# ylongqi/openrec

Hardware: NVIDIA H100
Metric: bpr_triplets_per_sec (higher is better)
Workload: dtype f32

## Files before the change

### include/orx.h

```cpp
#ifndef ORX_H_
#define ORX_H_

#include <stdint.h>

#ifdef __cplusplus
extern "C" {
#endif

#define ORX_ABI_VERSION 1
#define ORX_API __attribute__((visibility("default")))

typedef struct orx_ctx* orx_handle_t;
typedef void* orx_stream_t;

enum orx_status {
  ORX_OK = 0,
  ORX_ERR_INVALID = -1,
  ORX_ERR_CUDA = -2,
  ORX_ERR_UNSUPPORTED = -3,
  ORX_ERR_NOMEM = -4
};

enum orx_pair_kind { ORX_PAIR_BPR = 0, ORX_PAIR_UCML = 1 };
enum orx_point_kind { ORX_POINT_GMF = 0, ORX_POINT_WRMF = 1 };
// ... 26 lines not shown
  ORX_OP_GEMM = 0,
  ORX_OP_INTERACT_FWD = 1,
  ORX_OP_INTERACT_BWD = 2,
  ORX_OP_PAIRWISE_STEP = 3,
  ORX_OP_POINTWISE_STEP = 4,
  ORX_OP_SCORE_RANK = 5,
  ORX_OP_SCORE_TOPK = 6,
  ORX_OP_SCORE_RANK_SHARD = 7
};
enum orx_dispatch_variant {
  ORX_VARIANT_GEMM_TMA = 0,
  ORX_VARIANT_GEMM_SIMT = 1,
  ORX_VARIANT_INTERACT_WARP = 2,
  ORX_VARIANT_INTERACT = 3,
  ORX_VARIANT_STEP = 4,
  ORX_VARIANT_STEP_PIPE = 5,
  ORX_VARIANT_STEP_GENERIC = 6,
  ORX_VARIANT_RANK_SMEM = 7,
  ORX_VARIANT_RANK_GLOBAL = 8,
  ORX_VARIANT_TOPK = 9
};
#define ORX_DISPATCH_LOG_CAP 64
ORX_API int orx_debug_dispatch_log(orx_handle_t h, int32_t* rec_host, int32_t cap, int32_t* n_host);

ORX_API int orx_profile_enable(orx_handle_t h, int32_t on);
ORX_API int orx_profile_read(orx_handle_t h, float* ms_host, int32_t n_phases, int32_t* n_steps_host);

ORX_API int orx_fill_uniform(orx_handle_t h, float* dst, int64_t n, float lo, float hi, uint64_t seed, orx_stream_t s);
ORX_API int orx_gather(orx_handle_t h, const float* tab, int64_t rows, int32_t dim, const void* ids, int32_t id_is_i64,
               int64_t n, float* out, int32_t* n_bad, orx_stream_t s);
ORX_API int orx_censor(orx_handle_t h, float* tab, int64_t rows, int32_t dim, const int32_t* ids, int32_t n,
               float min_norm, orx_stream_t s);

ORX_API int orx_pairwise_step(orx_handle_t h, int32_t kind, const orx_table_t* user, const orx_table_t* item,
                      const orx_table_t* item_bias, const int32_t* uid, const int32_t* pid, const int32_t* nid,
                      int32_t B, float margin, float c_loss, float c_l2, const orx_opt_t* opt_host,
                      float* out4, orx_stream_t s);
ORX_API int orx_pairwise_step_host(orx_handle_t h, int32_t kind, const orx_table_t* user, const orx_table_t* item,
                           const orx_table_t* item_bias, const int32_t* uid_host, const int32_t* pid_host,
                           const int32_t* nid_host, int32_t B, float margin, float c_loss, float c_l2,
                           const orx_opt_t* opt_host, float* out4_host, orx_stream_t s);
ORX_API int orx_pairwise_prefetch(orx_handle_t h, const orx_table_t* user, const orx_table_t* item, const int32_t* uid,
                                  const int32_t* pid, const int32_t* nid, int32_t B, int32_t opt_kind, int32_t ids_ready,
                                  orx_stream_t ids_stream);
ORX_API int orx_pairwise_fwd(orx_handle_t h, int32_t kind, const orx_table_t* user, const orx_table_t* item,
                     const orx_table_t* item_bias, const int32_t* uid, const int32_t* pid, const int32_t* nid,
// ... 124 lines not shown
```

### openrec_b200/_lib.py

```python
from __future__ import annotations

import ctypes as C
import os

HERE = os.path.dirname(os.path.abspath(__file__))
LIB_PATH = os.path.join(HERE, "csrc", "liborx.so")

ORX_PAIR_BPR, ORX_PAIR_UCML = 0, 1
ORX_POINT_GMF, ORX_POINT_WRMF = 0, 1
ORX_SCORE_DOT, ORX_SCORE_NEG_SQDIST = 0, 1
ORX_OPT_SGD, ORX_OPT_ADAGRAD, ORX_OPT_ADAM_LAZY, ORX_OPT_ADAM_DENSE = 0, 1, 2, 3
ORX_OP_GEMM, ORX_OP_INTERACT_FWD, ORX_OP_INTERACT_BWD, ORX_OP_PAIRWISE_STEP, ORX_OP_POINTWISE_STEP = 0, 1, 2, 3, 4
ORX_OP_SCORE_RANK, ORX_OP_SCORE_TOPK, ORX_OP_SCORE_RANK_SHARD = 5, 6, 7
ORX_VARIANT_GEMM_TMA, ORX_VARIANT_GEMM_SIMT, ORX_VARIANT_INTERACT_WARP, ORX_VARIANT_INTERACT = 0, 1, 2, 3
ORX_VARIANT_STEP, ORX_VARIANT_STEP_PIPE, ORX_VARIANT_STEP_GENERIC = 4, 5, 6
ORX_VARIANT_RANK_SMEM, ORX_VARIANT_RANK_GLOBAL, ORX_VARIANT_TOPK = 7, 8, 9
ORX_MAX_AT = 8
ORX_MAX_TOPK = 1024
ORX_DISPATCH_LOG_CAP = 64


class OrxOpt(C.Structure):
    _fields_ = [("kind", C.c_int32), ("lr", C.c_float), ("eps", C.c_float), ("beta1", C.c_float),
                ("beta2", C.c_float), ("step", C.c_int64)]
# ... 16 lines not shown
                ("local_users", C.c_int64), ("local_items", C.c_int64)]


class OrxSampler(C.Structure):
    _fields_ = [("rec_user", C.c_void_p), ("rec_item", C.c_void_p), ("perm_cur", C.c_void_p), ("perm_next", C.c_void_p),
                ("cursor", C.c_int64), ("n_records", C.c_int64), ("csr_off", C.c_void_p), ("csr_items", C.c_void_p),
                ("total_users", C.c_int32), ("total_items", C.c_int32)]


_vp, _i32, _i64, _f, _u64 = C.c_void_p, C.c_int32, C.c_int64, C.c_float, C.c_uint64
_T = C.POINTER(OrxTable)
_O = C.POINTER(OrxOpt)
_S = C.POINTER(OrxShard)

SIGNATURES = {
    "orx_abi_version": [],
    "orx_last_error_string": [],
    "orx_create": [C.c_int, C.POINTER(_vp)],
    "orx_destroy": [_vp],
    "orx_device_count": [C.POINTER(C.c_int)],
    "orx_stream_synchronize": [_vp, _vp],
    "orx_debug_set_epoch": [_vp, C.c_uint32],
    "orx_debug_dispatch_log": [_vp, C.POINTER(_i32), _i32, C.POINTER(_i32)],
    "orx_profile_enable": [_vp, _i32],
    "orx_profile_read": [_vp, C.POINTER(C.c_float), _i32, C.POINTER(_i32)],
    "orx_fill_uniform": [_vp, _vp, _i64, _f, _f, _u64, _vp],
    "orx_gather": [_vp, _vp, _i64, _i32, _vp, _i32, _i64, _vp, _vp, _vp],
    "orx_censor": [_vp, _vp, _i64, _i32, _vp, _i32, _f, _vp],
    "orx_pairwise_step": [_vp, _i32, _T, _T, _T, _vp, _vp, _vp, _i32, _f, _f, _f, _O, _vp, _vp],
    "orx_pairwise_step_host": [_vp, _i32, _T, _T, _T, _vp, _vp, _vp, _i32, _f, _f, _f, _O, _vp, _vp],
    "orx_pairwise_prefetch": [_vp, _T, _T, _vp, _vp, _vp, _i32, _i32, _i32, _vp],
    "orx_pairwise_fwd": [_vp, _i32, _T, _T, _T, _vp, _vp, _vp, _i32, _f, _vp, _vp],
    "orx_pairwise_grad": [_vp, _i32, _T, _T, _T, _vp, _vp, _vp, _i32, _f, _f, _f, _vp, _vp, _vp, _vp, _vp, _vp, _vp],
    "orx_sparse_apply": [_vp, _T, _vp, _vp, _i32, _O, _vp],
    "orx_sparse_apply_strided": [_vp, _T, _vp, _i64, _vp, _i64, _i32, _O, _vp],
    "orx_gather_strided": [_vp, _vp, _i64, _i32, _vp, _i64, _i64, _vp, _i64, _vp, _vp],
    "orx_mlp_layer_fwd": [_vp, _vp, _i64, _i32, _i32, _vp, _vp, _i32, _i32, _vp, _i64, _vp],
    "orx_mlp_layer_bwd": [_vp, _vp, _i64, _vp, _i64, _vp, _i32, _i32, _i32, _i32, _vp, _i64, _vp, _i64, _vp, _vp, _vp],
    "orx_interact_fwd": [_vp, _vp, _i64, _vp, _i64, _i32, _i32, _i32, _i32, _i32, _vp, _i64, _vp],
    "orx_interact_bwd": [_vp, _vp, _i64, _vp, _i64, _vp, _i64, _i32, _i32, _i32, _i32, _i32, _vp, _i64, _vp, _i64,
                         _vp],
    "orx_pred_loss": [_vp, _vp, _vp, _i32, _i32, _f, _vp, _vp, _vp, _vp],
    "orx_peer_alloc": [_vp, _i64, C.POINTER(_vp), C.c_char_p],
    "orx_peer_open": [_vp, C.c_char_p, C.POINTER(_vp)],
    "orx_peer_close": [_vp, _vp],
    "orx_peer_free": [_vp, _vp],
# ... 51 lines not shown
```

### openrec_b200/csrc/orx_common.cuh

```cuda
#pragma once
#include <cuda_runtime.h>
#include <stdint.h>
#include <stdio.h>

#include <functional>
#include <initializer_list>
#include <type_traits>

#include "../../include/orx.h"

void orx_set_error(const char* fmt, ...);

#define ORX_CUDA(call)                                                                         \
  do {                                                                                         \
    cudaError_t e__ = (call);                                                                  \
    if (e__ != cudaSuccess) {                                                                  \
      orx_set_error("%s:%d %s -> %s", __FILE__, __LINE__, #call, cudaGetErrorString(e__));     \
      return ORX_ERR_CUDA;                                                                     \
    }                                                                                          \
  } while (0)

#define ORX_REQUIRE(cond, msg)                                  \
  do {                                                          \
    if (!(cond)) {                                              \
// ... 21 lines not shown
  OrxHash hu, hi;
  OrxHash pf_u[2], pf_i[2];
  int32_t* counters;
  float *gu, *gi, *gb, *gw;
  int64_t g_rows_u, g_rows_i;
  int32_t g_dim;
  float* partials;
  size_t partials_cap;
  int32_t* ids_stage[2];
  size_t stage_cap[2];
  float* out_stage[2];
  uint32_t stage_flip;
  int prof_on, prof_n, prof_cap;
  int prof_step;
  cudaEvent_t* prof_ev;
  int32_t* bucket_cursor;
  cudaStream_t side_stream;
  cudaEvent_t side_ev;
  cudaEvent_t pf_done[2], pf_free[2], stage_free[2];
  int pf_free_valid[2], stage_free_valid[2];
  int pf_valid, pf_set, pf_next, pf_B, pf_mode;
  const int32_t *pf_uid, *pf_pid, *pf_nid;
  int64_t pf_rows_u, pf_rows_i;
  uint32_t epoch;
  void* shard_ws;
  void* shard_scratch;
  size_t shard_cap;
  int32_t dispatch[ORX_DISPATCH_LOG_CAP][8];
  int64_t dispatch_n;
  void* eval_ws;
  size_t eval_cap;
  float* splitk;
  size_t splitk_cap;
};

int orx_grow(void** buf, size_t* cap, size_t need);

static inline void orx_log_dispatch(orx_ctx* c, int op, int variant, int TA, int TB, int M, int N, int K, int S) {
  int32_t* r = c->dispatch[c->dispatch_n++ % ORX_DISPATCH_LOG_CAP];
  r[0] = op; r[1] = variant; r[2] = TA; r[3] = TB; r[4] = M; r[5] = N; r[6] = K; r[7] = S;
}

int orx_next_epoch(orx_ctx* c, cudaStream_t st);
void orx_shard_ws_release(orx_ctx* c);
bool orx_shard_holds_index(const orx_ctx* c);

// ... 370 lines not shown
        if (!ZERO_ONLY) orx_update1<OPT>(W + e, P0 + e, P1 + e, W[e], G[e], a.opt);
        G[e] = 0.f;
      }
    }
    if (on && !is_u && sl == 0) {
      if (!ZERO_ONLY) orx_update1<OPT>(a.Bv + id, a.Bs0 + id, a.Bs1 + id, a.Bv[id], a.gb[d], a.opt);
      a.gb[d] = 0.f;
    }
  }
}
#endif

OrxOptDev orx_opt_to_dev(const orx_opt_t* o);
int orx_launch_index_build_strided(orx_ctx* c, const int32_t* a, int64_t stride, int64_t rows, int32_t n,
                                   bool stage_all, cudaStream_t st);
SparseArgs orx_sparse_args(const orx_ctx* c, const orx_table_t* user, const orx_table_t* item, const orx_table_t* bias,
                           const OrxHash& hu, const OrxHash& hi, const OrxOptDev& o);
int orx_check_step_tables(const orx_table_t* user, const orx_table_t* item, const orx_table_t* bias,
                          const orx_table_t* w, int opt_kind);
static inline int orx_step_blocks(int B) { return ((B + 7) / 8 + 7) / 8; }
struct OrxStepLaunch {
  int n_partials, variant, minb;
};
typedef std::function<int(const SparseArgs& s, float* partials, OrxStepLaunch* out)> OrxStepKernel;
int orx_sparse_step(orx_ctx* c, int op, int kind, const orx_table_t* user, const orx_table_t* item,
                    const orx_table_t* bias, const orx_table_t* w, const int32_t* uid, const int32_t* iid,
                    const int32_t* nid, int B, const orx_opt_t* opt, float loss_scale, float c_l2, float* out4,
                    const OrxStepKernel& kernel, cudaStream_t st);
int orx_sparse_unfused(orx_ctx* c, int B, float loss_scale, float* out4,
                       const std::function<void(float* partials, int blocks)>& launch, cudaStream_t st);
int orx_launch_adam_sweeps(orx_ctx* c, const orx_table_t* user, const orx_table_t* item, const orx_table_t* bias,
                           const OrxHash& hu, const OrxHash& hi, const OrxOptDev& o, cudaStream_t st);
int orx_launch_tail(orx_ctx* c, const TailArgs& ta, int opt_kind, cudaStream_t st);
int orx_launch_reduce_partials(const float* partials, int n, float loss_scale, float* out4, cudaStream_t st);
int orx_launch_index_build(orx_ctx* c, const int32_t* a, int64_t rows_a, const int32_t* b0, const int32_t* b1,
                           int64_t rows_b, int32_t n, int mode , cudaStream_t st);
```

### openrec_b200/csrc/orx_ctx.cu

```cuda
#include <stdarg.h>
#include <stdlib.h>
#include <string.h>

#include "orx_common.cuh"

static thread_local char g_err[512] = "";

void orx_set_error(const char* fmt, ...) {
  va_list ap;
  va_start(ap, fmt);
  vsnprintf(g_err, sizeof(g_err), fmt, ap);
  va_end(ap);
}

extern "C" const char* orx_last_error_string(void) { return g_err; }

bool orx_pdl_enabled() {
  static int v = -1;
  if (v < 0) {
    const char* e = getenv("ORX_PDL");
    v = (e && atoi(e) == 0) ? 0 : 1;
  }
  return v != 0;
}
// ... 51 lines not shown
  return ORX_OK;
}

int orx_ensure_workspace(orx_ctx* c, int64_t B, int32_t dim) {
  if (B <= c->cap_B && dim <= c->g_dim) return ORX_OK;
  if (orx_shard_holds_index(c)) {
    orx_set_error("workspace growth to %lld lookups / dim %d refused: a sharded step's announced batch holds this "
                  "handle's index sets until its orx_shard_step call", (long long)B, dim);
    return ORX_ERR_INVALID;
  }
  int64_t nb = B > c->cap_B ? B : c->cap_B;
  int32_t nd = dim > c->g_dim ? dim : c->g_dim;
  ORX_CUDA(cudaDeviceSynchronize());
  free_workspace(c);
  int rc;
  if ((rc = alloc_hash(c->hu, nb, c->counters + 0)) != ORX_OK) return rc;
  if ((rc = alloc_hash(c->hi, 2 * nb, c->counters + 1)) != ORX_OK) return rc;
  for (int k = 0; k < 2; ++k) {
    if ((rc = alloc_hash(c->pf_u[k], nb, c->counters + 4 * (1 + k))) != ORX_OK) return rc;
    if ((rc = alloc_hash(c->pf_i[k], 2 * nb, c->counters + 4 * (1 + k) + 1)) != ORX_OK) return rc;
  }
  c->pf_valid = 0;
  c->pf_free_valid[0] = c->pf_free_valid[1] = 0;
  c->g_rows_u = nb;
  c->g_rows_i = 2 * nb;
  size_t bu = sizeof(float) * (size_t)c->g_rows_u * nd, bi = sizeof(float) * (size_t)c->g_rows_i * nd;
  ORX_CUDA(cudaMalloc(&c->gu, bu));
  ORX_CUDA(cudaMalloc(&c->gi, bi));
  ORX_CUDA(cudaMalloc(&c->gb, sizeof(float) * (size_t)c->g_rows_i));
  ORX_CUDA(cudaMalloc(&c->gw, sizeof(float) * (size_t)nd));
  ORX_CUDA(cudaMemset(c->gu, 0, bu));
  ORX_CUDA(cudaMemset(c->gi, 0, bi));
  ORX_CUDA(cudaMemset(c->gb, 0, sizeof(float) * (size_t)c->g_rows_i));
  ORX_CUDA(cudaMemset(c->gw, 0, sizeof(float) * (size_t)nd));
  ORX_CUDA(cudaMemset(c->counters, 0, sizeof(int32_t) * 16));
  ORX_CUDA(cudaDeviceSynchronize());
  c->cap_B = nb;
  c->g_dim = nd;
  c->epoch = 0;
  return ORX_OK;
}

static int zero_hash(OrxHash& t) {
  if (!t.slots) return ORX_OK;
  ORX_CUDA(cudaMemset(t.slots, 0, sizeof(unsigned long long) * ((size_t)t.mask + 1)));
  return ORX_OK;
// ... 52 lines not shown
  *cap = need;
  return ORX_OK;
}

extern "C" int orx_create(int device, orx_handle_t* out) {
  ORX_REQUIRE(out != nullptr, "null output handle");
  *out = nullptr;
  int n = 0;
  ORX_CUDA(cudaGetDeviceCount(&n));
  ORX_REQUIRE(device >= 0 && device < n, "device ordinal out of range");
  ORX_CUDA(cudaSetDevice(device));
  cudaDeviceProp prop;
  ORX_CUDA(cudaGetDeviceProperties(&prop, device));
  if (prop.major != 9 || prop.minor != 0) {
    orx_set_error("orx_create: liborx is built for sm_90a only; device %d is sm_%d%d", device, prop.major,
                  prop.minor);
    return ORX_ERR_UNSUPPORTED;
  }
  orx_ctx* c = new orx_ctx();
  memset(c, 0, sizeof(*c));
  c->device = device;
  c->num_sms = prop.multiProcessorCount;
  c->partials_cap = sizeof(float) * 2 * (size_t)c->num_sms * 64;
  if (cudaMalloc(&c->counters, sizeof(int32_t) * 16) != cudaSuccess ||
      cudaMalloc(&c->bucket_cursor, sizeof(int32_t) * 1024) != cudaSuccess ||
      cudaMalloc(&c->partials, c->partials_cap) != cudaSuccess ||
      cudaMalloc(&c->out_stage[0], sizeof(float) * 8) != cudaSuccess ||
      cudaMalloc(&c->out_stage[1], sizeof(float) * 8) != cudaSuccess) {
    orx_set_error("orx_create: workspace allocation failed: %s", cudaGetErrorString(cudaGetLastError()));
    orx_destroy(c);
    return ORX_ERR_NOMEM;
  }
  cudaMemset(c->counters, 0, sizeof(int32_t) * 16);
  *out = c;
  return ORX_OK;
}

extern "C" int orx_destroy(orx_handle_t h) {
  if (!h) return ORX_OK;
  cudaSetDevice(h->device);
  cudaDeviceSynchronize();
  free_workspace(h);
  for (int i = 0; i < 2; ++i) {
    cudaFree(h->ids_stage[i]);
    cudaFree(h->out_stage[i]);
  }
  cudaFree(h->counters);
  cudaFree(h->partials);
  cudaFree(h->bucket_cursor);
  cudaFree(h->eval_ws);
  cudaFree(h->splitk);
  cudaFree(h->shard_scratch);
  orx_shard_ws_release(h);
  if (h->side_stream) {
    cudaStreamDestroy(h->side_stream);
    cudaEventDestroy(h->side_ev);
    for (int i = 0; i < 2; ++i) {
      cudaEventDestroy(h->pf_done[i]);
      cudaEventDestroy(h->pf_free[i]);
      cudaEventDestroy(h->stage_free[i]);
    }
  }
  if (h->prof_ev) {
    for (int i = 0; i < h->prof_cap * ORX_PROF_EV; ++i) cudaEventDestroy(h->prof_ev[i]);
    delete[] h->prof_ev;
  }
  delete h;
  return ORX_OK;
// ... 60 lines not shown
```

### openrec_b200/csrc/orx_pair.cuh

```cuda
#pragma once
#include "orx_common.cuh"

struct PairArgs : SparseArgs {
  int64_t rowsU, rowsI;
  const int32_t *uid, *pid, *nid;
  int B;
  float margin, c_loss, c_l2, inv_B;
  float* partials;
  float *d_user, *d_pos, *d_neg, *d_bp, *d_bn, *g_out;
  int64_t ld;
};

__device__ __forceinline__ float dot4(float4 a, float4 b) { return a.x * b.x + a.y * b.y + a.z * b.z + a.w * b.w; }
__device__ __forceinline__ float sqd4(float4 a, float4 b) {
  float x = a.x - b.x, y = a.y - b.y, z = a.z - b.z, w = a.w - b.w;
  return x * x + y * y + z * z + w * w;
}
__device__ __forceinline__ float4 axmb_pcd(float s, float4 a, float4 b, float c, float4 d) {
  return make_float4(s * (a.x - b.x) + c * d.x, s * (a.y - b.y) + c * d.y, s * (a.z - b.z) + c * d.z,
                     s * (a.w - b.w) + c * d.w);
}
__device__ __forceinline__ float4 sa_pcd(float s, float4 a, float c, float4 d) {
  return make_float4(s * a.x + c * d.x, s * a.y + c * d.y, s * a.z + c * d.z, s * a.w + c * d.w);
}

template <int KIND>
__device__ __forceinline__ void pair_score(float s1, float s2, float bp, float bn, float margin, float c_loss,
                                           float inv_B, float* loss_term, float* g) {
  if (KIND == ORX_PAIR_BPR) {
    const float x = (s1 + bp) - (s2 + bn);
    const float y = fmaxf(x, -30.f);
// ... 42 lines not shown
```

### openrec_b200/csrc/orx_pairwise.cu

```cuda
#include "orx_common.cuh"
#include "orx_pair.cuh"

__global__ void k_index_build(OrxHash hu, OrxHash hi, const int32_t* __restrict__ a, int64_t rows_a,
                              const int32_t* __restrict__ b0, const int32_t* __restrict__ b1, int64_t rows_b, int n,
                              int stage_all, int32_t* bad) {
  const int i = blockIdx.x * blockDim.x + threadIdx.x;
  if (i >= (b1 ? 3 : 2) * n) return;
  const int t = i < n ? i : (i < 2 * n ? i - n : i - 2 * n);
  const int32_t ia = a[t], ib0 = b0[t], ib1 = b1 ? b1[t] : 0;
  const bool ga = ia >= 0 && (int64_t)ia < rows_a, gb0 = ib0 >= 0 && (int64_t)ib0 < rows_b,
             gb1 = ib1 >= 0 && (int64_t)ib1 < rows_b;
  const bool all = ga && gb0 && gb1;
  if (i < n) {
    if (!ga) atomicAdd(bad, 1);
    else if (all) orx_hash_insert(hu, ia, stage_all);
  } else {
    const bool g = i < 2 * n ? gb0 : gb1;
    if (!g) atomicAdd(bad, 1);
    else if (all) orx_hash_insert(hi, i < 2 * n ? ib0 : ib1, stage_all);
  }
}

__global__ void k_index_build_strided(OrxHash hu, const int32_t* __restrict__ a, int64_t stride, int64_t rows, int n,
                                       int stage_all, int32_t* bad) {
  for (int i = blockIdx.x * blockDim.x + threadIdx.x; i < n; i += gridDim.x * blockDim.x) {
    const int32_t id = a[(int64_t)i * stride];
    if (id >= 0 && (int64_t)id < rows) orx_hash_insert(hu, id, stage_all);
    else atomicAdd(bad, 1);
  }
}

int orx_launch_index_build_strided(orx_ctx* c, const int32_t* a, int64_t stride, int64_t rows, int32_t n,
                                   bool stage_all, cudaStream_t st) {
  if (n <= 0) return ORX_OK;
  int rc = orx_next_epoch(c, st);
  if (rc) return rc;
  k_index_build_strided<<<(n + 255) / 256, 256, 0, st>>>(c->hu, a, stride, rows, n, stage_all ? 1 : 0, c->counters + 3);
  ORX_LAUNCH_CHECK();
  return ORX_OK;
}

int orx_launch_index_build(orx_ctx* c, const int32_t* a, int64_t rows_a, const int32_t* b0, const int32_t* b1,
                           int64_t rows_b, int32_t n, int mode, cudaStream_t st) {
  const int total = (b1 ? 3 : 2) * n;
  if (total <= 0) return ORX_OK;
  int rc = orx_next_epoch(c, st);
  if (rc) return rc;
  k_index_build<<<(total + 255) / 256, 256, 0, st>>>(c->hu, c->hi, a, rows_a, b0, b1, rows_b, n, mode, c->counters + 3);
  ORX_LAUNCH_CHECK();
  return ORX_OK;
}

template <int K, bool S0, bool S1>
struct TripRegs {
  float4 u[K], p[K], n[K];
  float4 us0[K], ps0[K], ns0[K];
  float4 us1[K], ps1[K], ns1[K];
  int fl, uu, pp, nn, du, dp, dn;
  float bp, bn;
};

template <int KIND, int OPT, int D, int CH, int MINB, bool PIPE>
__global__ void __launch_bounds__(256, MINB) k_pair_step(const PairArgs a) {
  constexpr int G = (D / 4 < 32) ? D / 4 : 32;
  constexpr int K = D / (4 * G);
  constexpr int TPW = 32 / G;
  typedef OrxOptSlots<OPT> SL;
  static_assert(CH % TPW == 0, "chunk must be a multiple of the triplets per warp");
  typedef TripRegs<K, SL::S0, SL::S1> Regs;

  const int lane = threadIdx.x & 31;
  const int warp = (blockIdx.x * blockDim.x + threadIdx.x) >> 5;
  const int grp = lane / G, gl = lane % G;
  const int t = warp * CH + lane;
  const float4 z4 = make_float4(0.f, 0.f, 0.f, 0.f);
  orx_pdl_wait();

  int u_id = 0, p_id = 0, n_id = 0, du = -1, dp = -1, dn = -1, flags = 0;
  if (lane < CH && t < a.B) {
    u_id = a.uid[t];
    p_id = a.pid[t];
    n_id = a.nid[t];
    flags = (u_id >= 0 && u_id < a.rowsU && p_id >= 0 && p_id < a.rowsI && n_id >= 0 && n_id < a.rowsI) ? 1 : 0;
  }

  auto load_var = [&](int j, Regs& r) {
    const int src = j + grp;
    r.fl = __shfl_sync(ORX_FULL, flags, src) & 1;
    r.uu = __shfl_sync(ORX_FULL, u_id, src);
    r.pp = __shfl_sync(ORX_FULL, p_id, src);
    r.nn = __shfl_sync(ORX_FULL, n_id, src);
#pragma unroll
    for (int k = 0; k < K; ++k) {
      const int off = (k * G + gl) * 4;
      r.u[k] = r.fl ? orx_ld4_stream(a.U + (int64_t)r.uu * D + off) : z4;
      r.p[k] = r.fl ? orx_ld4_stream(a.I + (int64_t)r.pp * D + off) : z4;
      r.n[k] = r.fl ? orx_ld4_stream(a.I + (int64_t)r.nn * D + off) : z4;
    }
  };
  Regs ra, rb;
  load_var(0, ra);
  if (PIPE && TPW < CH) load_var(TPW, rb);

  float bp = 0.f, bn = 0.f, bps0 = 0.f, bps1 = 0.f, bns0 = 0.f, bns1 = 0.f;
  if (flags & 1) {
    const uint32_t cu = orx_hash_find<!SL::STAGE_ONLY, true>(a.hu, u_id, &du);
    const uint32_t cp = orx_hash_find<!SL::STAGE_ONLY, true>(a.hi, p_id, &dp);
    const uint32_t cn = orx_hash_find<!SL::STAGE_ONLY, true>(a.hi, n_id, &dn);
    bp = orx_ld_keep(a.Bv + p_id);
    bn = orx_ld_keep(a.Bv + n_id);
    if (!SL::STAGE_ONLY) {
      flags |= (cu == 1u ? 2 : 0) | (cp == 1u ? 4 : 0) | (cn == 1u ? 8 : 0);
      if (SL::S0) {
        if (flags & 4) bps0 = orx_ld_keep(a.Bs0 + p_id);
        if (flags & 8) bns0 = orx_ld_keep(a.Bs0 + n_id);
      }
      if (SL::S1) {
        if (flags & 4) bps1 = orx_ld_keep(a.Bs1 + p_id);
        if (flags & 8) bns1 = orx_ld_keep(a.Bs1 + n_id);
      }
    }
  }

  auto load_slots = [&](int j, Regs& r) {
    const int src = j + grp;
    r.fl = __shfl_sync(ORX_FULL, flags, src);
    r.du = __shfl_sync(ORX_FULL, du, src);
    r.dp = __shfl_sync(ORX_FULL, dp, src);
    r.dn = __shfl_sync(ORX_FULL, dn, src);
    r.bp = __shfl_sync(ORX_FULL, bp, src);
    r.bn = __shfl_sync(ORX_FULL, bn, src);
#pragma unroll
    for (int k = 0; k < K; ++k) {
      const int off = (k * G + gl) * 4;
      if (SL::S0) {
        r.us0[k] = (r.fl & 2) ? orx_ld4_stream(a.Us0 + (int64_t)r.uu * D + off) : z4;
        r.ps0[k] = (r.fl & 4) ? orx_ld4_stream(a.Is0 + (int64_t)r.pp * D + off) : z4;
        r.ns0[k] = (r.fl & 8) ? orx_ld4_stream(a.Is0 + (int64_t)r.nn * D + off) : z4;
      }
      if (SL::S1) {
        r.us1[k] = (r.fl & 2) ? orx_ld4_stream(a.Us1 + (int64_t)r.uu * D + off) : z4;
        r.ps1[k] = (r.fl & 4) ? orx_ld4_stream(a.Is1 + (int64_t)r.pp * D + off) : z4;
        r.ns1[k] = (r.fl & 8) ? orx_ld4_stream(a.Is1 + (int64_t)r.nn * D + off) : z4;
      }
    }
  };
  load_slots(0, ra);
  if (PIPE && TPW < CH) load_slots(TPW, rb);

  float loss_acc = 0.f, l2_acc = 0.f, g_own = 0.f;

  auto process = [&](int j, Regs& r) {
    float s1 = 0.f, s2 = 0.f, sq = 0.f;
#pragma unroll
    for (int k = 0; k < K; ++k) {
      if (KIND == ORX_PAIR_BPR) {
        s1 += dot4(r.u[k], r.p[k]);
        s2 += dot4(r.u[k], r.n[k]);
      } else {
        s1 += sqd4(r.u[k], r.p[k]);
        s2 += sqd4(r.u[k], r.n[k]);
      }
      sq += dot4(r.u[k], r.u[k]) + dot4(r.p[k], r.p[k]) + dot4(r.n[k], r.n[k]);
    }
    l2_acc += sq;
    s1 = orx_group_sum<G>(s1);
    s2 = orx_group_sum<G>(s2);
    float lt, g;
    pair_score<KIND>(s1, s2, r.bp, r.bn, a.margin, a.c_loss, a.inv_B, &lt, &g);
    const bool v = r.fl & 1;
    if (!v) { lt = 0.f; g = 0.f; }
    if (gl == 0) loss_acc += lt;
    const float gbias = (KIND == ORX_PAIR_BPR) ? g : -g;
#pragma unroll
    for (int q = 0; q < TPW; ++q) {
      const float val = __shfl_sync(ORX_FULL, gbias, q * G);
      if (lane == j + q) g_own = val;
    }
    if (v) {
#pragma unroll
      for (int k = 0; k < K; ++k) {
        const int off = (k * G + gl) * 4;
        float4 gu, gp, gn;
        pair_row_grads<KIND>(g, a.c_l2, r.u[k], r.p[k], r.n[k], &gu, &gp, &gn);
        orx_own_or_stage4<OPT, true>(r.fl & 2, a.U, a.Us0, a.Us1, r.uu, a.gu, r.du, D, off, r.u[k], gu, r.us0[k],
                                     r.us1[k], a.opt);
        orx_own_or_stage4<OPT, true>(r.fl & 4, a.I, a.Is0, a.Is1, r.pp, a.gi, r.dp, D, off, r.p[k], gp, r.ps0[k],
                                     r.ps1[k], a.opt);
        orx_own_or_stage4<OPT, true>(r.fl & 8, a.I, a.Is0, a.Is1, r.nn, a.gi, r.dn, D, off, r.n[k], gn, r.ns0[k],
                                     r.ns1[k], a.opt);
      }
    }
// ... 290 lines not shown
static int prefetch_drop(orx_ctx* c, cudaStream_t st) {
  if (!c->pf_valid) return ORX_OK;
  const int k = c->pf_set;
  ORX_CUDA(cudaStreamWaitEvent(st, c->pf_done[k], 0));
  ORX_CUDA(cudaMemsetAsync(c->counters + 4 * (1 + k), 0, sizeof(int32_t) * 4, st));
  ORX_CUDA(cudaEventRecord(c->pf_free[k], st));
  c->pf_free_valid[k] = 1;
  c->pf_valid = 0;
  return ORX_OK;
}

static int prefetch_issue(orx_ctx* c, const int32_t* uid, const int32_t* pid, const int32_t* nid, int B, int64_t rows_u,
                          int64_t rows_i, int mode) {
  const int k = c->pf_next;
  c->pf_next ^= 1;
  cudaStream_t ss = c->side_stream;
  if (c->pf_free_valid[k]) ORX_CUDA(cudaStreamWaitEvent(ss, c->pf_free[k], 0));
  int rc = orx_next_epoch(c, ss);
  if (rc) return rc;
  c->pf_u[k].epoch = c->pf_i[k].epoch = c->epoch;
  k_index_build<<<(3 * B + 255) / 256, 256, 0, ss>>>(c->pf_u[k], c->pf_i[k], uid, rows_u, pid, nid, rows_i, B, mode,
                                                     c->counters + 4 * (1 + k) + 3);
  ORX_LAUNCH_CHECK();
  ORX_CUDA(cudaEventRecord(c->pf_done[k], ss));
  c->pf_valid = 1; c->pf_set = k; c->pf_uid = uid; c->pf_pid = pid; c->pf_nid = nid; c->pf_B = B;
  c->pf_rows_u = rows_u; c->pf_rows_i = rows_i; c->pf_mode = mode;
  return ORX_OK;
}

extern "C" int orx_pairwise_prefetch(orx_handle_t h, const orx_table_t* user, const orx_table_t* item, const int32_t* uid,
                                     const int32_t* pid, const int32_t* nid, int32_t B, int32_t opt_kind, int32_t ids_ready,
                                     orx_stream_t ids_stream) {
  ORX_REQUIRE(h != nullptr && user && item && uid && pid && nid && B > 0, "bad arguments");
  ORX_REQUIRE(orx_opt_kind_ok(opt_kind), "unknown optimizer kind");
  ORX_REQUIRE(!orx_shard_holds_index(h), "a sharded step's announced batch holds this handle's index sets (a prefetch "
                                         "would overwrite one) until its orx_shard_step call");
  ORX_CUDA(cudaSetDevice(h->device));
  cudaStream_t is = (cudaStream_t)ids_stream;
  int rc = orx_ensure_workspace(h, B, user->dim);
  if (rc) return rc;
  if ((rc = side_stream_ensure(h))) return rc;
  if ((rc = prefetch_drop(h, is))) return rc;
  if (!ids_ready) {
    ORX_CUDA(cudaEventRecord(h->side_ev, is));
    ORX_CUDA(cudaStreamWaitEvent(h->side_stream, h->side_ev, 0));
  }
  return prefetch_issue(h, uid, pid, nid, B, user->rows, item->rows, opt_kind == ORX_OPT_ADAM_DENSE ? 1 : 0);
}

int orx_sparse_step(orx_ctx* c, int op, int kind, const orx_table_t* user, const orx_table_t* item,
                    const orx_table_t* bias, const orx_table_t* w, const int32_t* uid, const int32_t* iid,
                    const int32_t* nid, int B, const orx_opt_t* opt, float loss_scale, float c_l2, float* out4,
                    const OrxStepKernel& kernel, cudaStream_t st) {
  ORX_REQUIRE(opt != nullptr && out4 != nullptr, "null opt/out");
  ORX_REQUIRE(orx_opt_kind_ok(opt->kind), "unknown optimizer kind");
  ORX_REQUIRE(B > 0 && uid && iid, "empty batch or null ids");
  int rc = orx_check_step_tables(user, item, bias, w, opt->kind);
  if (rc) return rc;
  const int D = user->dim;
  if ((rc = orx_ensure_workspace(c, B, D))) return rc;
  const bool dense = opt->kind == ORX_OPT_ADAM_DENSE;
  if ((rc = orx_grow((void**)&c->partials, &c->partials_cap, sizeof(float) * 2 * 8 * (size_t)orx_step_blocks(B))))
    return rc;
  orx_prof_mark(c, 0, st);
  int set = 0;
  if (nid && c->pf_valid && c->pf_uid == uid && c->pf_pid == iid && c->pf_nid == nid && c->pf_B == B &&
      c->pf_rows_u == user->rows && c->pf_rows_i == item->rows && c->pf_mode == (dense ? 1 : 0)) {
    set = 1 + c->pf_set;
    ORX_CUDA(cudaStreamWaitEvent(st, c->pf_done[c->pf_set], 0));
    c->pf_valid = 0;
  } else {
    if (nid && (rc = prefetch_drop(c, st))) return rc;
    if ((rc = orx_launch_index_build(c, uid, user->rows, iid, nid, item->rows, B, dense ? 1 : 0, st))) return rc;
  }
  const OrxHash& HU = set ? c->pf_u[set - 1] : c->hu;
  const OrxHash& HI = set ? c->pf_i[set - 1] : c->hi;
  orx_prof_mark(c, 1, st);
  const SparseArgs s = orx_sparse_args(c, user, item, bias, HU, HI, orx_opt_to_dev(opt));
  OrxStepLaunch L = {};
  if ((rc = kernel(s, c->partials, &L))) return rc;
  orx_log_dispatch(c, op, L.variant, kind, opt->kind, B, D, L.minb, set);
  orx_prof_mark(c, 2, st);
  if (dense && (rc = orx_launch_adam_sweeps(c, user, item, bias, HU, HI, s.opt, st))) return rc;
  TailArgs ta = {s};
  ta.partials = c->partials; ta.n_partials = L.n_partials; ta.loss_scale = loss_scale;
  ta.counters = c->counters + 4 * set; ta.out4 = out4;
  if (w) {
    ta.W = w->var; ta.Ws0 = w->s0; ta.Ws1 = w->s1; ta.gw = c->gw; ta.c_l2 = c_l2;
  }
  rc = orx_launch_tail(c, ta, opt->kind, st);
  if (set) {
    ORX_CUDA(cudaEventRecord(c->pf_free[set - 1], st));
    c->pf_free_valid[set - 1] = 1;
  }
  orx_prof_mark(c, 3, st);
  orx_prof_next(c);
  return rc;
}

static PairArgs pair_args(const SparseArgs& s, int64_t rows_u, int64_t rows_i, const int32_t* uid, const int32_t* pid,
                          const int32_t* nid, int B, float margin, float c_loss, float c_l2, float inv_B) {
  PairArgs pa = {s};
  pa.rowsU = rows_u; pa.rowsI = rows_i;
  pa.uid = uid; pa.pid = pid; pa.nid = nid; pa.B = B;
  pa.margin = margin; pa.c_loss = c_loss; pa.c_l2 = c_l2; pa.inv_B = inv_B;
  return pa;
}

static int pairwise_step_impl(orx_ctx* c, int kind, const orx_table_t* user, const orx_table_t* item,
                              const orx_table_t* bias, const int32_t* uid, const int32_t* pid, const int32_t* nid,
                              int B, float margin, float c_loss, float c_l2, const orx_opt_t* opt, float* out4,
                              cudaStream_t st) {
  ORX_REQUIRE(kind == ORX_PAIR_BPR || kind == ORX_PAIR_UCML, "unknown pairwise kind");
  ORX_REQUIRE(nid != nullptr, "empty batch or null ids");
  const float inv_B = 1.0f / (float)B;
  const auto kernel = [&](const SparseArgs& s, float* partials, OrxStepLaunch* out) {
    PairArgs pa = pair_args(s, user->rows, item->rows, uid, pid, nid, B, margin, c_loss, c_l2, inv_B);
    pa.partials = partials;
    return orx_dispatch<ORX_PAIR_BPR, ORX_PAIR_UCML>(kind, [&](auto K) {
      return orx_dispatch_opt(opt->kind, [&](auto O) {
        return launch_pair_step_kind_opt<decltype(K)::value, decltype(O)::value>(pa, st, out);
      });
    });
  };
  return orx_sparse_step(c, ORX_OP_PAIRWISE_STEP, kind, user, item, bias, nullptr, uid, pid, nid, B, opt,
                         kind == ORX_PAIR_BPR ? inv_B : 1.0f, c_l2, out4, kernel, st);
}

extern "C" int orx_pairwise_step(orx_handle_t h, int32_t kind, const orx_table_t* user, const orx_table_t* item,
                                 const orx_table_t* item_bias, const int32_t* uid, const int32_t* pid,
                                 const int32_t* nid, int32_t B, float margin, float c_loss, float c_l2,
                                 const orx_opt_t* opt, float* out4, orx_stream_t s) {
  ORX_REQUIRE(h != nullptr, "null handle");
  ORX_CUDA(cudaSetDevice(h->device));
  return pairwise_step_impl(h, kind, user, item, item_bias, uid, pid, nid, B, margin, c_loss, c_l2, opt, out4,
                            (cudaStream_t)s);
}

extern "C" int orx_pairwise_step_host(orx_handle_t h, int32_t kind, const orx_table_t* user, const orx_table_t* item,
                                      const orx_table_t* item_bias, const int32_t* uid_host, const int32_t* pid_host,
                                      const int32_t* nid_host, int32_t B, float margin, float c_loss, float c_l2,
// ... 120 lines not shown
```

### openrec_b200/csrc/orx_pointwise.cu

```cuda
#include "orx_common.cuh"

struct PointArgs : SparseArgs {
  const float* W;
  float* gw;
  int64_t rowsU, rowsI;
  const int32_t *uid, *iid;
  const float* label;
  int B;
  float wa, wb, c_loss, c_l2, inv_B;
  int use_sigmoid;
  float* partials;
  float *d_user, *d_item, *d_bias, *g_out;
};

template <int KIND>
__device__ __forceinline__ void point_score(float s, float bias, float label, const PointArgs& a, float* lt,
                                            float* g) {
  if (KIND == ORX_POINT_GMF) {
    const float z = s + bias;
    *lt = fmaxf(z, 0.f) - z * label + log1pf(expf(-fabsf(z)));
    *g = a.c_loss * (orx_sigmoid(z) - label) * a.inv_B;
  } else {
    float pred = s + bias;
    if (a.use_sigmoid) pred = orx_sigmoid(pred);
// ... 246 lines not shown
                            const orx_table_t* item, const int32_t* uid, const int32_t* iid, const float* label, int B,
                            float a, float b, int use_sigmoid, float c_loss, float c_l2) {
  PointArgs pa = {s};
  pa.W = dense_w ? dense_w->var : nullptr;
  pa.rowsU = user->rows; pa.rowsI = item->rows;
  pa.uid = uid; pa.iid = iid; pa.label = label; pa.B = B;
  pa.wa = a; pa.wb = b; pa.c_loss = c_loss; pa.c_l2 = c_l2; pa.inv_B = 1.0f / (float)B;
  pa.use_sigmoid = use_sigmoid;
  return pa;
}

extern "C" int orx_pointwise_step(orx_handle_t h, int32_t kind, const orx_table_t* user, const orx_table_t* item,
                                  const orx_table_t* item_bias, const orx_table_t* w, const int32_t* uid,
                                  const int32_t* iid, const float* label, int32_t B, float a, float b,
                                  int32_t use_sigmoid, float c_loss, float c_l2, const orx_opt_t* opt, float* out4,
                                  orx_stream_t s) {
  ORX_REQUIRE(h != nullptr, "null handle");
  ORX_REQUIRE(label != nullptr, "empty batch or null inputs");
  ORX_REQUIRE(kind == ORX_POINT_GMF || kind == ORX_POINT_WRMF, "unknown pointwise kind");
  ORX_REQUIRE(kind == ORX_POINT_WRMF || w, "GMF needs w with dim == D");
  const orx_table_t* dense_w = (kind == ORX_POINT_GMF) ? w : nullptr;
  ORX_CUDA(cudaSetDevice(h->device));
  cudaStream_t st = (cudaStream_t)s;
  const auto kernel = [&](const SparseArgs& sa, float* partials, OrxStepLaunch* out) {
    PointArgs pa = point_args(sa, dense_w, user, item, uid, iid, label, B, a, b, use_sigmoid, c_loss, c_l2);
    pa.partials = partials;
    pa.gw = dense_w ? h->gw : nullptr;
    return orx_dispatch<ORX_POINT_GMF, ORX_POINT_WRMF>(kind, [&](auto K) {
      return orx_dispatch_opt(opt->kind, [&](auto O) {
        return launch_point_kind_opt<decltype(K)::value, decltype(O)::value>(pa, st, out);
      });
    });
  };
  return orx_sparse_step(h, ORX_OP_POINTWISE_STEP, kind, user, item, item_bias, dense_w, uid, iid, nullptr, B, opt,
                         dense_w ? 1.0f / (float)B : 1.0f, c_l2, out4, kernel, st);
}

static int point_fwd_grad(orx_ctx* h, int kind, const orx_table_t* user, const orx_table_t* item,
                          const orx_table_t* bias, const orx_table_t* w, const int32_t* uid, const int32_t* iid,
                          const float* label, int B, float a, float b, int use_sigmoid, float c_loss, float c_l2,
                          float* d_user, float* d_item, float* d_bias, float* d_w, float* g_out, float* out4,
                          cudaStream_t st) {
  ORX_REQUIRE(B > 0 && uid && iid && label, "empty batch or null inputs");
  ORX_REQUIRE(kind == ORX_POINT_GMF || kind == ORX_POINT_WRMF, "unknown pointwise kind");
  ORX_REQUIRE(kind == ORX_POINT_WRMF || w, "GMF needs w with dim == D");
  const orx_table_t* dense_w = (kind == ORX_POINT_GMF) ? w : nullptr;
  int rc = orx_check_step_tables(user, item, bias, dense_w, ORX_OPT_SGD);
// ... 43 lines not shown
```

### openrec_b200/native.py

```python
from __future__ import annotations

import ctypes as C
from collections import namedtuple

import torch

from . import _lib
from ._lib import (ORX_OP_GEMM, ORX_OP_INTERACT_BWD, ORX_OP_INTERACT_FWD, ORX_OP_PAIRWISE_STEP, ORX_OP_POINTWISE_STEP,
                   ORX_OP_SCORE_RANK, ORX_OP_SCORE_RANK_SHARD, ORX_OP_SCORE_TOPK, ORX_OPT_ADAGRAD, ORX_OPT_ADAM_DENSE, ORX_OPT_ADAM_LAZY, ORX_OPT_SGD, ORX_PAIR_BPR,
                   ORX_PAIR_UCML, ORX_POINT_GMF, ORX_POINT_WRMF, ORX_SCORE_DOT, ORX_SCORE_NEG_SQDIST, ORX_VARIANT_GEMM_SIMT,
                   ORX_VARIANT_GEMM_TMA, ORX_VARIANT_INTERACT, ORX_VARIANT_INTERACT_WARP, ORX_VARIANT_RANK_GLOBAL,
                   ORX_VARIANT_RANK_SMEM, ORX_VARIANT_STEP, ORX_VARIANT_STEP_GENERIC, ORX_VARIANT_STEP_PIPE,
                   ORX_VARIANT_TOPK, OrxOpt, OrxTable)

__all__ = ["Engine", "engine", "table", "opt", "ORX_PAIR_BPR", "ORX_PAIR_UCML", "ORX_POINT_GMF", "ORX_POINT_WRMF",
           "ORX_OPT_SGD", "ORX_OPT_ADAGRAD", "ORX_OPT_ADAM_LAZY", "ORX_OPT_ADAM_DENSE", "ORX_SCORE_DOT",
           "ORX_SCORE_NEG_SQDIST", "ORX_OP_GEMM", "ORX_OP_INTERACT_FWD", "ORX_OP_INTERACT_BWD", "ORX_OP_PAIRWISE_STEP",
           "ORX_OP_POINTWISE_STEP", "ORX_VARIANT_GEMM_TMA", "ORX_VARIANT_GEMM_SIMT", "ORX_VARIANT_INTERACT_WARP",
           "ORX_VARIANT_INTERACT", "ORX_VARIANT_STEP", "ORX_VARIANT_STEP_PIPE", "ORX_VARIANT_STEP_GENERIC",
           "ORX_OP_SCORE_RANK", "ORX_VARIANT_RANK_SMEM", "ORX_VARIANT_RANK_GLOBAL", "ORX_OP_SCORE_TOPK",
           "ORX_VARIANT_TOPK", "ORX_OP_SCORE_RANK_SHARD", "Dispatch", "RowShard", "rowshard"]

_engines = {}

# ... 104 lines not shown
                                              _ptr(out4), self.stream()), "orx_pairwise_step")

    def pairwise_step_host(self, kind, user, item, bias, uid_h, pid_h, nid_h, o, out4_h, margin=0.5, c_loss=1.0,
                           c_l2=1.0):
        _lib.check(self.lib.orx_pairwise_step_host(self.h, kind, C.byref(user), C.byref(item), C.byref(bias),
                                                   _ptr(uid_h), _ptr(pid_h), _ptr(nid_h), uid_h.numel(), margin,
                                                   c_loss, c_l2, C.byref(o), _ptr(out4_h), self.stream()),
                   "orx_pairwise_step_host")

    def pairwise_prefetch(self, user, item, uid, pid, nid, opt_kind, ids_ready=False):
        _lib.check(self.lib.orx_pairwise_prefetch(self.h, C.byref(user), C.byref(item), _ptr(uid), _ptr(pid), _ptr(nid),
                                                  uid.numel(), opt_kind, 1 if ids_ready else 0, self.stream()),
                   "orx_pairwise_prefetch")

    def debug_set_epoch(self, epoch):
        _lib.check(self.lib.orx_debug_set_epoch(self.h, epoch), "orx_debug_set_epoch")

    def debug_dispatch_log(self):
        rec = (C.c_int32 * (8 * _lib.ORX_DISPATCH_LOG_CAP))()
        n = C.c_int32()
        _lib.check(self.lib.orx_debug_dispatch_log(self.h, rec, _lib.ORX_DISPATCH_LOG_CAP, C.byref(n)),
                   "orx_debug_dispatch_log")
        return [Dispatch(*rec[8 * i:8 * i + 8]) for i in range(n.value)]

    def pairwise_fwd(self, kind, user, item, bias, uid, pid, nid, out4, margin=0.5):
        _lib.check(self.lib.orx_pairwise_fwd(self.h, kind, C.byref(user), C.byref(item), C.byref(bias), _ptr(uid),
                                             _ptr(pid), _ptr(nid), uid.numel(), margin, _ptr(out4), self.stream()),
                   "orx_pairwise_fwd")

    def pairwise_grad(self, kind, user, item, bias, uid, pid, nid, margin=0.5, c_loss=1.0, c_l2=1.0, *, d_user=None,
                      d_pos=None, d_neg=None, d_bp=None, d_bn=None, g_out=None):
        _lib.check(self.lib.orx_pairwise_grad(self.h, kind, C.byref(user), C.byref(item), C.byref(bias), _ptr(uid),
                                              _ptr(pid), _ptr(nid), uid.numel(), margin, c_loss, c_l2, _ptr(d_user),
                                              _ptr(d_pos), _ptr(d_neg), _ptr(d_bp), _ptr(d_bn), _ptr(g_out),
                                              self.stream()), "orx_pairwise_grad")

    def sparse_apply(self, tab, ids, values, o):
        n = 0 if ids is None else ids.numel()
        _lib.check(self.lib.orx_sparse_apply(self.h, C.byref(tab), _ptr(ids), _ptr(values), n, C.byref(o),
                                             self.stream()), "orx_sparse_apply")

    def sparse_apply_strided(self, tab, ids2d, col, values3d, o):
        n, F = ids2d.shape
        D = values3d.shape[2]
        _lib.check(self.lib.orx_sparse_apply_strided(
            self.h, C.byref(tab), C.c_void_p(ids2d.data_ptr() + 4 * col), F,
# ... 184 lines not shown
```

Baseline: 353.9 million.

## Precompute hash-slot resolution per triplet on prefetch stream for pairwise step

Adds a resolve kernel that runs on the side prefetch stream after the index build. It looks up the user, positive and negative hash slots for every triplet and stores them with validity and first-occurrence flags as an int4 record. The main pairwise step kernel then reads that record instead of doing three hash probes and bounds checks, which moves latency-bound probing off the critical path. In exchange it writes and reads an extra 16 bytes per triplet and launches one more kernel on the side stream. It also stops shuffling the item biases in the register struct and reads them by shuffle at use time, and adds a debug API to read the records back.

```diff
diff --git a/include/orx.h b/include/orx.h
--- a/include/orx.h
+++ b/include/orx.h
@@ -72,6 +72,7 @@
 };
 #define ORX_DISPATCH_LOG_CAP 64
 ORX_API int orx_debug_dispatch_log(orx_handle_t h, int32_t* rec_host, int32_t cap, int32_t* n_host);
+ORX_API int orx_debug_pair_records(orx_handle_t h, int32_t set, int32_t* rec, int32_t B, orx_stream_t stream);
 
 ORX_API int orx_profile_enable(orx_handle_t h, int32_t on);
 ORX_API int orx_profile_read(orx_handle_t h, float* ms_host, int32_t n_phases, int32_t* n_steps_host);
diff --git a/openrec_b200/_lib.py b/openrec_b200/_lib.py
--- a/openrec_b200/_lib.py
+++ b/openrec_b200/_lib.py
@@ -62,6 +62,7 @@
     "orx_stream_synchronize": [_vp, _vp],
     "orx_debug_set_epoch": [_vp, C.c_uint32],
     "orx_debug_dispatch_log": [_vp, C.POINTER(_i32), _i32, C.POINTER(_i32)],
+    "orx_debug_pair_records": [_vp, _i32, _vp, _i32, _vp],
     "orx_profile_enable": [_vp, _i32],
     "orx_profile_read": [_vp, C.POINTER(C.c_float), _i32, C.POINTER(_i32)],
     "orx_fill_uniform": [_vp, _vp, _i64, _f, _f, _u64, _vp],
diff --git a/openrec_b200/csrc/orx_common.cuh b/openrec_b200/csrc/orx_common.cuh
--- a/openrec_b200/csrc/orx_common.cuh
+++ b/openrec_b200/csrc/orx_common.cuh
@@ -67,6 +67,9 @@
   int pf_valid, pf_set, pf_next, pf_B, pf_mode;
   const int32_t *pf_uid, *pf_pid, *pf_nid;
   int64_t pf_rows_u, pf_rows_i;
+  int4* pf_res[2];
+  size_t pf_res_cap[2];
+  int pair_resolve;
   uint32_t epoch;
   void* shard_ws;
   void* shard_scratch;
@@ -483,7 +486,7 @@
 struct OrxStepLaunch {
   int n_partials, variant, minb;
 };
-typedef std::function<int(const SparseArgs& s, float* partials, OrxStepLaunch* out)> OrxStepKernel;
+typedef std::function<int(const SparseArgs& s, const int4* res, float* partials, OrxStepLaunch* out)> OrxStepKernel;
 int orx_sparse_step(orx_ctx* c, int op, int kind, const orx_table_t* user, const orx_table_t* item,
                     const orx_table_t* bias, const orx_table_t* w, const int32_t* uid, const int32_t* iid,
                     const int32_t* nid, int B, const orx_opt_t* opt, float loss_scale, float c_l2, float* out4,
diff --git a/openrec_b200/csrc/orx_ctx.cu b/openrec_b200/csrc/orx_ctx.cu
--- a/openrec_b200/csrc/orx_ctx.cu
+++ b/openrec_b200/csrc/orx_ctx.cu
@@ -97,6 +97,8 @@
   }
   c->pf_valid = 0;
   c->pf_free_valid[0] = c->pf_free_valid[1] = 0;
+  for (int k = 0; k < 2 && c->pair_resolve; ++k)
+    if ((rc = orx_grow((void**)&c->pf_res[k], &c->pf_res_cap[k], sizeof(int4) * (size_t)nb)) != ORX_OK) return rc;
   c->g_rows_u = nb;
   c->g_rows_i = 2 * nb;
   size_t bu = sizeof(float) * (size_t)c->g_rows_u * nd, bi = sizeof(float) * (size_t)c->g_rows_i * nd;
@@ -195,6 +197,8 @@
   c->device = device;
   c->num_sms = prop.multiProcessorCount;
   c->partials_cap = sizeof(float) * 2 * (size_t)c->num_sms * 64;
+  const char* pr = getenv("ORX_PAIR_RESOLVE");
+  c->pair_resolve = (pr && atoi(pr) == 0) ? 0 : 1;
   if (cudaMalloc(&c->counters, sizeof(int32_t) * 16) != cudaSuccess ||
       cudaMalloc(&c->bucket_cursor, sizeof(int32_t) * 1024) != cudaSuccess ||
       cudaMalloc(&c->partials, c->partials_cap) != cudaSuccess ||
@@ -217,6 +221,7 @@
   for (int i = 0; i < 2; ++i) {
     cudaFree(h->ids_stage[i]);
     cudaFree(h->out_stage[i]);
+    cudaFree(h->pf_res[i]);
   }
   cudaFree(h->counters);
   cudaFree(h->partials);
diff --git a/openrec_b200/csrc/orx_pair.cuh b/openrec_b200/csrc/orx_pair.cuh
--- a/openrec_b200/csrc/orx_pair.cuh
+++ b/openrec_b200/csrc/orx_pair.cuh
@@ -7,6 +7,7 @@
   int B;
   float margin, c_loss, c_l2, inv_B;
   float* partials;
+  const int4* res;
   float *d_user, *d_pos, *d_neg, *d_bp, *d_bn, *g_out;
   int64_t ld;
 };
diff --git a/openrec_b200/csrc/orx_pairwise.cu b/openrec_b200/csrc/orx_pairwise.cu
--- a/openrec_b200/csrc/orx_pairwise.cu
+++ b/openrec_b200/csrc/orx_pairwise.cu
@@ -21,6 +21,29 @@
   }
 }
 
+__global__ void k_index_resolve(OrxHash hu, OrxHash hi, const int32_t* __restrict__ uid, const int32_t* __restrict__ pid,
+                                const int32_t* __restrict__ nid, int64_t rows_u, int64_t rows_i, int n, int mode,
+                                int4* __restrict__ res) {
+  const int t = blockIdx.x * blockDim.x + threadIdx.x;
+  if (t >= n) return;
+  const int32_t u = uid[t], p = pid[t], q = nid[t];
+  int4 r = make_int4(0, -1, -1, -1);
+  if (u >= 0 && (int64_t)u < rows_u && p >= 0 && (int64_t)p < rows_i && q >= 0 && (int64_t)q < rows_i) {
+    if (mode == 1) {
+      orx_hash_find(hu, u, &r.y);
+      orx_hash_find(hi, p, &r.z);
+      orx_hash_find(hi, q, &r.w);
+      r.x = 1;
+    } else {
+      const uint32_t cu = orx_hash_find<true>(hu, u, &r.y);
+      const uint32_t cp = orx_hash_find<true>(hi, p, &r.z);
+      const uint32_t cn = orx_hash_find<true>(hi, q, &r.w);
+      r.x = 1 | (cu == 1u ? 2 : 0) | (cp == 1u ? 4 : 0) | (cn == 1u ? 8 : 0);
+    }
+  }
+  res[t] = r;
+}
+
 __global__ void k_index_build_strided(OrxHash hu, const int32_t* __restrict__ a, int64_t stride, int64_t rows, int n,
                                        int stage_all, int32_t* bad) {
   for (int i = blockIdx.x * blockDim.x + threadIdx.x; i < n; i += gridDim.x * blockDim.x) {
@@ -57,7 +80,6 @@
   float4 us0[K], ps0[K], ns0[K];
   float4 us1[K], ps1[K], ns1[K];
   int fl, uu, pp, nn, du, dp, dn;
-  float bp, bn;
 };
 
 template <int KIND, int OPT, int D, int CH, int MINB, bool PIPE>
@@ -81,7 +103,15 @@
     u_id = a.uid[t];
     p_id = a.pid[t];
     n_id = a.nid[t];
-    flags = (u_id >= 0 && u_id < a.rowsU && p_id >= 0 && p_id < a.rowsI && n_id >= 0 && n_id < a.rowsI) ? 1 : 0;
+    if (a.res) {
+      const int4 r = __ldcs(a.res + t);
+      flags = r.x;
+      du = r.y;
+      dp = r.z;
+      dn = r.w;
+    } else {
+      flags = (u_id >= 0 && u_id < a.rowsU && p_id >= 0 && p_id < a.rowsI && n_id >= 0 && n_id < a.rowsI) ? 1 : 0;
+    }
   }
 
   auto load_var = [&](int j, Regs& r) {
@@ -104,13 +134,16 @@
 
   float bp = 0.f, bn = 0.f, bps0 = 0.f, bps1 = 0.f, bns0 = 0.f, bns1 = 0.f;
   if (flags & 1) {
-    const uint32_t cu = orx_hash_find<!SL::STAGE_ONLY, true>(a.hu, u_id, &du);
-    const uint32_t cp = orx_hash_find<!SL::STAGE_ONLY, true>(a.hi, p_id, &dp);
-    const uint32_t cn = orx_hash_find<!SL::STAGE_ONLY, true>(a.hi, n_id, &dn);
+    uint32_t cu = 0, cp = 0, cn = 0;
+    if (!a.res) {
+      cu = orx_hash_find<!SL::STAGE_ONLY, true>(a.hu, u_id, &du);
+      cp = orx_hash_find<!SL::STAGE_ONLY, true>(a.hi, p_id, &dp);
+      cn = orx_hash_find<!SL::STAGE_ONLY, true>(a.hi, n_id, &dn);
+    }
     bp = orx_ld_keep(a.Bv + p_id);
     bn = orx_ld_keep(a.Bv + n_id);
     if (!SL::STAGE_ONLY) {
-      flags |= (cu == 1u ? 2 : 0) | (cp == 1u ? 4 : 0) | (cn == 1u ? 8 : 0);
+      if (!a.res) flags |= (cu == 1u ? 2 : 0) | (cp == 1u ? 4 : 0) | (cn == 1u ? 8 : 0);
       if (SL::S0) {
         if (flags & 4) bps0 = orx_ld_keep(a.Bs0 + p_id);
         if (flags & 8) bns0 = orx_ld_keep(a.Bs0 + n_id);
@@ -128,8 +161,6 @@
     r.du = __shfl_sync(ORX_FULL, du, src);
     r.dp = __shfl_sync(ORX_FULL, dp, src);
     r.dn = __shfl_sync(ORX_FULL, dn, src);
-    r.bp = __shfl_sync(ORX_FULL, bp, src);
-    r.bn = __shfl_sync(ORX_FULL, bn, src);
 #pragma unroll
     for (int k = 0; k < K; ++k) {
       const int off = (k * G + gl) * 4;
@@ -167,7 +198,8 @@
     s1 = orx_group_sum<G>(s1);
     s2 = orx_group_sum<G>(s2);
     float lt, g;
-    pair_score<KIND>(s1, s2, r.bp, r.bn, a.margin, a.c_loss, a.inv_B, &lt, &g);
+    pair_score<KIND>(s1, s2, __shfl_sync(ORX_FULL, bp, j + grp), __shfl_sync(ORX_FULL, bn, j + grp), a.margin, a.c_loss,
+                     a.inv_B, &lt, &g);
     const bool v = r.fl & 1;
     if (!v) { lt = 0.f; g = 0.f; }
     if (gl == 0) loss_acc += lt;
@@ -504,6 +536,11 @@
   k_index_build<<<(3 * B + 255) / 256, 256, 0, ss>>>(c->pf_u[k], c->pf_i[k], uid, rows_u, pid, nid, rows_i, B, mode,
                                                      c->counters + 4 * (1 + k) + 3);
   ORX_LAUNCH_CHECK();
+  if (c->pair_resolve) {
+    k_index_resolve<<<(B + 255) / 256, 256, 0, ss>>>(c->pf_u[k], c->pf_i[k], uid, pid, nid, rows_u, rows_i, B, mode,
+                                                      c->pf_res[k]);
+    ORX_LAUNCH_CHECK();
+  }
   ORX_CUDA(cudaEventRecord(c->pf_done[k], ss));
   c->pf_valid = 1; c->pf_set = k; c->pf_uid = uid; c->pf_pid = pid; c->pf_nid = nid; c->pf_B = B;
   c->pf_rows_u = rows_u; c->pf_rows_i = rows_i; c->pf_mode = mode;
@@ -528,6 +565,16 @@
     ORX_CUDA(cudaStreamWaitEvent(h->side_stream, h->side_ev, 0));
   }
   return prefetch_issue(h, uid, pid, nid, B, user->rows, item->rows, opt_kind == ORX_OPT_ADAM_DENSE ? 1 : 0);
+}
+
+extern "C" int orx_debug_pair_records(orx_handle_t h, int32_t set, int32_t* rec, int32_t B, orx_stream_t s) {
+  ORX_REQUIRE(h != nullptr && rec && (set == 1 || set == 2) && B > 0, "bad arguments");
+  ORX_REQUIRE(h->pair_resolve && h->side_stream && sizeof(int4) * (size_t)B <= h->pf_res_cap[set - 1],
+              "no records of that many triplets (ORX_PAIR_RESOLVE=0, no prefetch yet, or B beyond the workspace)");
+  ORX_CUDA(cudaSetDevice(h->device));
+  ORX_CUDA(cudaStreamWaitEvent((cudaStream_t)s, h->pf_done[set - 1], 0));
+  ORX_CUDA(cudaMemcpyAsync(rec, h->pf_res[set - 1], sizeof(int4) * (size_t)B, cudaMemcpyDeviceToDevice, (cudaStream_t)s));
+  return ORX_OK;
 }
 
 int orx_sparse_step(orx_ctx* c, int op, int kind, const orx_table_t* user, const orx_table_t* item,
@@ -560,7 +607,7 @@
   orx_prof_mark(c, 1, st);
   const SparseArgs s = orx_sparse_args(c, user, item, bias, HU, HI, orx_opt_to_dev(opt));
   OrxStepLaunch L = {};
-  if ((rc = kernel(s, c->partials, &L))) return rc;
+  if ((rc = kernel(s, set && c->pair_resolve ? c->pf_res[set - 1] : nullptr, c->partials, &L))) return rc;
   orx_log_dispatch(c, op, L.variant, kind, opt->kind, B, D, L.minb, set);
   orx_prof_mark(c, 2, st);
   if (dense && (rc = orx_launch_adam_sweeps(c, user, item, bias, HU, HI, s.opt, st))) return rc;
@@ -596,9 +643,10 @@
   ORX_REQUIRE(kind == ORX_PAIR_BPR || kind == ORX_PAIR_UCML, "unknown pairwise kind");
   ORX_REQUIRE(nid != nullptr, "empty batch or null ids");
   const float inv_B = 1.0f / (float)B;
-  const auto kernel = [&](const SparseArgs& s, float* partials, OrxStepLaunch* out) {
+  const auto kernel = [&](const SparseArgs& s, const int4* res, float* partials, OrxStepLaunch* out) {
     PairArgs pa = pair_args(s, user->rows, item->rows, uid, pid, nid, B, margin, c_loss, c_l2, inv_B);
     pa.partials = partials;
+    pa.res = res;
     return orx_dispatch<ORX_PAIR_BPR, ORX_PAIR_UCML>(kind, [&](auto K) {
       return orx_dispatch_opt(opt->kind, [&](auto O) {
         return launch_pair_step_kind_opt<decltype(K)::value, decltype(O)::value>(pa, st, out);
diff --git a/openrec_b200/csrc/orx_pointwise.cu b/openrec_b200/csrc/orx_pointwise.cu
--- a/openrec_b200/csrc/orx_pointwise.cu
+++ b/openrec_b200/csrc/orx_pointwise.cu
@@ -292,7 +292,7 @@
   const orx_table_t* dense_w = (kind == ORX_POINT_GMF) ? w : nullptr;
   ORX_CUDA(cudaSetDevice(h->device));
   cudaStream_t st = (cudaStream_t)s;
-  const auto kernel = [&](const SparseArgs& sa, float* partials, OrxStepLaunch* out) {
+  const auto kernel = [&](const SparseArgs& sa, const int4* , float* partials, OrxStepLaunch* out) {
     PointArgs pa = point_args(sa, dense_w, user, item, uid, iid, label, B, a, b, use_sigmoid, c_loss, c_l2);
     pa.partials = partials;
     pa.gw = dense_w ? h->gw : nullptr;
diff --git a/openrec_b200/native.py b/openrec_b200/native.py
--- a/openrec_b200/native.py
+++ b/openrec_b200/native.py
@@ -150,6 +150,12 @@
         _lib.check(self.lib.orx_debug_dispatch_log(self.h, rec, _lib.ORX_DISPATCH_LOG_CAP, C.byref(n)),
                    "orx_debug_dispatch_log")
         return [Dispatch(*rec[8 * i:8 * i + 8]) for i in range(n.value)]
+
+    def debug_pair_records(self, index_set, B):
+        rec = torch.empty((B, 4), dtype=torch.int32, device=self.device)
+        _lib.check(self.lib.orx_debug_pair_records(self.h, index_set, _ptr(rec), B, self.stream()),
+                   "orx_debug_pair_records")
+        return rec
 
     def pairwise_fwd(self, kind, user, item, bias, uid, pid, nid, out4, margin=0.5):
         _lib.check(self.lib.orx_pairwise_fwd(self.h, kind, C.byref(user), C.byref(item), C.byref(bias), _ptr(uid),
```

Result: faster. 368.8 million, median of 6 (+4.2%).
